# 87003697/DynamiCrafter

Hardware: AMD Instinct MI355X
Metric: frames/sec (and denoising-step ms), 16f@576x1024, DDIM 50 (higher is better)
Workload: dtype bf16; 1 GPU; inference_1024_v1.0.yaml: 1 clip/GPU, 16 frames, latent 72x128, DDIM 50 uniform_trailing eta=1, CFG 7.5 batched (cond+uncond), guidance_rescale 0.7, v-param+ZTSNR+dynamic rescale, hipGraph-captured step; clips_per_gpu=1, parallelism=dp1 over 1 distinct clips (no data-path collective), conditioning=local (1 rank), outputs_finite=True

## Files before the change

### dynamicrafter_amd/_hip.py

```python
import ctypes as C
import os
import threading

_HERE = os.path.dirname(os.path.abspath(__file__))
LIB_PATH = os.environ.get("DC_HIP_LIB") or os.path.join(_HERE, "csrc", "libdcrafter_hip.so")

DC_GEMM_OUT_F32 = 1
DC_GEMM_GEGLU = 2
DC_GEMM_GELU = 4


class DcGemmParams(C.Structure):
    _fields_ = [
        ("A", C.c_void_p), ("W", C.c_void_p), ("C", C.c_void_p), ("bias", C.c_void_p),
        ("rowvec", C.c_void_p), ("residual", C.c_void_p),
        ("lda", C.c_int), ("ldc", C.c_int), ("ldr", C.c_int), ("rowvec_ld", C.c_int),
        ("rows_per_vec", C.c_int),
        ("M", C.c_int), ("N", C.c_int), ("K", C.c_int), ("n_pad", C.c_int),
        ("mode", C.c_int), ("Cin", C.c_int),
        ("IH", C.c_int), ("IW", C.c_int), ("OH", C.c_int), ("OW", C.c_int),
        ("stride", C.c_int), ("pad", C.c_int), ("ups", C.c_int),
        ("T", C.c_int), ("HW", C.c_int),
        ("flags", C.c_int), ("alpha", C.c_float),
        ("workspace", C.c_void_p), ("workspace_bytes", C.c_longlong),
    ]


class DcDdimParams(C.Structure):
    _fields_ = [
        ("a_t", C.c_void_p), ("a_prev", C.c_void_p), ("sigma_t", C.c_void_p), ("sqrt_one_minus_at", C.c_void_p),
        ("sqrt_acp_t", C.c_void_p), ("sqrt_1macp_t", C.c_void_p), ("scale_ratio", C.c_void_p),
        ("step_index", C.c_void_p),
        ("index", C.c_int), ("v_param", C.c_int),
        ("cfg_scale", C.c_float), ("cfg_img", C.c_float), ("guidance_rescale", C.c_float),
        ("temperature", C.c_float),
        ("e_nchw", C.c_int), ("noise_step_stride", C.c_int64),
    ]


class DcDpmParams(C.Structure):
    _fields_ = [
        ("A", C.c_void_p), ("alpha_t", C.c_void_p), ("alpha_p_r", C.c_void_p), ("k", C.c_void_p), ("N", C.c_void_p),
        ("sqrt_one_minus_at", C.c_void_p), ("sqrt_acp_t", C.c_void_p), ("sqrt_1macp_t", C.c_void_p),
        ("scale_ratio", C.c_void_p), ("step_index", C.c_void_p),
        ("index", C.c_int), ("v_param", C.c_int),
        ("cfg_scale", C.c_float), ("cfg_img", C.c_float), ("guidance_rescale", C.c_float),
        ("temperature", C.c_float),
# ... 125 lines not shown
```

### dynamicrafter_amd/csrc/gemm_conv_glds.hip

```cpp
#include "dc_common.h"
#include "dcrafter_hip.h"
#include "lds_stage.h"
#include <stdint.h>
#include <stdlib.h>
#include <type_traits>
#include <utility>

namespace {

constexpr int GBM = 256;
constexpr int GBK = 64;
constexpr int GNT = 512;

struct GemmSplit {
    float* partial;
    int splits;
    int tile_begin;
    int tile_count;
    int* err;
    int whole;
};

template <int BN, bool GEGLU, int MODE, int GSTAGES>
__global__ __launch_bounds__(GNT) void gemm_conv_glds_kernel(const DcGemmParams p, const GemmSplit sp) {
    constexpr int NB = BN / 64;
    constexpr int BNOUT = GEGLU ? BN / 2 : BN;
    constexpr int A_BYTES = GBM * GBK * 2;
    constexpr int B_BYTES = BN * GBK * 2;
    constexpr int STAGE = A_BYTES + B_BYTES;
    constexpr int A_IT = 4;
    constexpr int B_IT = BN / 64;
    constexpr int LOADS = A_IT + B_IT;
    static_assert(GSTAGES == 2 || GSTAGES == 3, "ring depth");
    static_assert(!GEGLU || (NB % 2 == 0), "GEGLU needs value and gate blocks per wave");
    extern __shared__ __attribute__((aligned(16))) char smem[];

    const int tid = threadIdx.x;
    const int lane = tid & 63;
    const int wave = __builtin_amdgcn_readfirstlane(tid >> 6);
    const int wm = wave >> 1, wn = wave & 1;

    const int n_out = GEGLU ? (p.N >> 1) : p.N;
    const int tiles_n = (n_out + BNOUT - 1) / BNOUT;
    const int tiles_m = (p.M + GBM - 1) / GBM;
// ... 264 lines not shown
                    const uint2 rr = *reinterpret_cast<const uint2*>(p.residual + (size_t)m * p.ldr + n);
                    const float a0 = __uint_as_float(pk.x << 16) + __uint_as_float(rr.x << 16);
                    const float a1 = __uint_as_float(pk.x & 0xffff0000u) + __uint_as_float(rr.x & 0xffff0000u);
                    const float a2 = __uint_as_float(pk.y << 16) + __uint_as_float(rr.y << 16);
                    const float a3 = __uint_as_float(pk.y & 0xffff0000u) + __uint_as_float(rr.y & 0xffff0000u);
                    pk.x = pack_bf2(a0, a1);
                    pk.y = pack_bf2(a2, a3);
                }
                *reinterpret_cast<uint2*>(reinterpret_cast<bf16_t*>(p.C) + (size_t)m * p.ldc + n) = pk;
            }
        }
    }
}

template <int BN>
__global__ __launch_bounds__(256) void splitk_reduce_kernel(const DcGemmParams p, const GemmSplit sp) {
    constexpr int UPR = BN / 4;
    const int tiles_n = (p.N + BN - 1) / BN;
    const int t_loc = blockIdx.y;
    const int u = blockIdx.x * 256 + threadIdx.x;
    if (u >= GBM * UPR) return;
    const int r = u / UPR, c = (u - r * UPR) * 4;
    const int tile = sp.tile_begin + t_loc;
    const int m = (tile / tiles_n) * GBM + r, n = (tile % tiles_n) * BN + c;
    if (m >= p.M || n >= p.N) return;
    float4 v = make_float4(0.f, 0.f, 0.f, 0.f);
    for (int s = 0; s < sp.splits; ++s) {
        const float4 a = *reinterpret_cast<const float4*>(sp.partial + (((size_t)s * sp.tile_count + t_loc) * GBM + r) * BN + c);
        v.x += a.x; v.y += a.y; v.z += a.z; v.w += a.w;
    }
    if (p.bias) {
        const float4 bv = *reinterpret_cast<const float4*>(p.bias + n);
        v.x += bv.x; v.y += bv.y; v.z += bv.z; v.w += bv.w;
    }
    if (p.flags & DC_GEMM_GELU) { v.x = DC_GELU(v.x); v.y = DC_GELU(v.y); v.z = DC_GELU(v.z); v.w = DC_GELU(v.w); }
    if (p.rowvec) {
        const float4 rv = *reinterpret_cast<const float4*>(p.rowvec + (size_t)(m / p.rows_per_vec) * p.rowvec_ld + n);
        v.x += rv.x; v.y += rv.y; v.z += rv.z; v.w += rv.w;
    }
    if (p.alpha != 1.0f) { v.x *= p.alpha; v.y *= p.alpha; v.z *= p.alpha; v.w *= p.alpha; }
    if (p.flags & DC_GEMM_OUT_F32) {
        *reinterpret_cast<float4*>(reinterpret_cast<float*>(p.C) + (size_t)m * p.ldc + n) = v;
        return;
    }
    uint2 pk;
    pk.x = pack_bf2(v.x, v.y);
    pk.y = pack_bf2(v.z, v.w);
// ... 457 lines not shown
}

constexpr int PLAN_DEFAULT = 3 | 16;
constexpr int PLAN_MASK = 3 | 16 | 32 | 64 | 128 | 256;
inline bool plan_valid(int plan) { return plan >= 0 && plan <= 511 && !(plan & 4); }
std::atomic<int> g_gemm_plan{[] {
    const char* e = getenv("DC_GEMM_PLAN");
    const int v = e ? atoi(e) : PLAN_DEFAULT;
    return plan_valid(v) ? (v & PLAN_MASK) : PLAN_DEFAULT;
}()};
inline int pipe_min_k() { static const int v = [] { const char* e = getenv("DC_PIPE_MIN_K"); return e ? atoi(e) : 1920; }(); return v; }

template <int MODE, int EPI>
int launch_pipe_shape(const DcGemmParams& p, hipStream_t stream, GemmSplit sp, int gx, int gy) {
    sp.err = dc_error_word_device();
    if (!sp.err) return DC_ERR_ARG;
    return launch_pipe320x16<MODE, EPI>(p, stream, sp, gx, gy);
}

inline bool pipe_ok(const DcGemmParams& p, int plan) {
    if (!(plan & 3) || (!(plan & 2) && p.mode != 1)) return false;
    if (p.mode != 1 && p.K < pipe_min_k()) return false;
    if (p.flags & (DC_GEMM_GEGLU | DC_GEMM_OUT_F32)) return false;
    if (p.ups && !(p.mode == 1 && p.ups == 1 && p.stride == 1 && p.pad == 1 && p.OH == 2 * p.IH && p.OW == 2 * p.IW)) return false;
    if (p.N % 320 != 0 || p.n_pad < p.N || p.K % 64 != 0 || p.lda % 8 != 0 || ((uintptr_t)p.A % 16) != 0) return false;
    if (p.ldc % 8 != 0 || ((uintptr_t)p.C % 16) != 0 || (long long)p.M * p.ldc >= (1ll << 31)) return false;
    if (p.residual && (p.ldr % 8 != 0 || ((uintptr_t)p.residual % 16) != 0 || (long long)p.M * p.ldr >= (1ll << 31))) return false;
    long long rows = p.M, extra = 0;
    if (p.mode == 1) { if (p.Cin % 64 != 0 || p.K != 9 * p.Cin) return false; rows = (long long)(p.M / (p.OH * p.OW) + 1) * p.IH * p.IW; extra = 2ll * p.IW + 2; }
    else if (p.mode == 2) { if (p.Cin % 64 != 0 || p.K != 3 * p.Cin) return false; extra = 2ll * p.HW; }
    else if (p.mode != 0) return false;
    if ((rows + extra) * p.lda * 2 >= (1ll << 31)) return false;
    if (320ll * p.K * 2 >= (1ll << 31)) return false;
    return true;
}

int launch_pipe_whole(const DcGemmParams& p, hipStream_t stream) {
    const int ntiles = ((p.M + GBM - 1) / GBM) * (p.N / 320);
    GemmSplit sp;
    sp.partial = nullptr; sp.splits = 1; sp.tile_begin = 0; sp.tile_count = ntiles; sp.err = nullptr; sp.whole = 0;
    dc_note_variant(p.mode == 0 ? "gemm_pipe320x16_kernel" : p.mode == 2 ? "gemm_pipe320x16_kernel<tconv>"
                    : p.ups ? "gemm_pipe320x16_kernel<conv,ups>" : "gemm_pipe320x16_kernel<conv>");
    if (p.mode == 0) return p.residual ? launch_pipe_shape<0, 1>(p, stream, sp, ntiles, 1) : launch_pipe_shape<0, 0>(p, stream, sp, ntiles, 1);
    if (p.mode == 1 && p.ups) return p.residual ? launch_pipe_shape<3, 1>(p, stream, sp, ntiles, 1) : launch_pipe_shape<3, 0>(p, stream, sp, ntiles, 1);
    if (p.mode == 1) return p.residual ? launch_pipe_shape<1, 1>(p, stream, sp, ntiles, 1) : launch_pipe_shape<1, 0>(p, stream, sp, ntiles, 1);
    return p.residual ? launch_pipe_shape<2, 1>(p, stream, sp, ntiles, 1) : launch_pipe_shape<2, 0>(p, stream, sp, ntiles, 1);
}

template <int MODE, int BN = 320>
int launch_glds320_split(const DcGemmParams& p, hipStream_t stream, int ntiles, int full, int splits, bool use_pipe, bool merged) {
    constexpr int GSTAGES = 2;
    constexpr size_t lds = (size_t)GSTAGES * (GBM * GBK * 2 + BN * GBK * 2);
    static DcLdsOnce lds_once;
    if (const int e = lds_once.ensure(reinterpret_cast<const void*>(&gemm_conv_glds_kernel<BN, false, MODE, GSTAGES>), (int)lds)) return e;
    if constexpr (BN == 320) {
        if (use_pipe) {
            dc_note_variant(MODE == 0 ? "gemm_pipe320x16_kernel+splitk" : MODE == 2 ? "gemm_pipe320x16_kernel<tconv>+splitk"
                            : MODE == 3 ? "gemm_pipe320x16_kernel<conv,ups>+splitk" : "gemm_pipe320x16_kernel<conv>+splitk");
            GemmSplit sp;
            sp.err = nullptr; sp.whole = 0;
            if (full > 0 && merged && full % 8 == 0) {
                sp.partial = reinterpret_cast<float*>(p.workspace); sp.splits = splits; sp.tile_begin = full; sp.tile_count = ntiles - full;
                sp.whole = full;
                const int gx = full + sp.tile_count * splits;
                if (const int e = p.residual ? launch_pipe_shape<MODE, 1>(p, stream, sp, gx, 1) : launch_pipe_shape<MODE, 0>(p, stream, sp, gx, 1)) return e;
                sp.whole = 0;
            } else {
                if (full > 0) {
                    sp.partial = nullptr; sp.splits = 1; sp.tile_begin = 0; sp.tile_count = full;
                    if (const int e = p.residual ? launch_pipe_shape<MODE, 1>(p, stream, sp, full, 1) : launch_pipe_shape<MODE, 0>(p, stream, sp, full, 1)) return e;
                }
                sp.partial = reinterpret_cast<float*>(p.workspace); sp.splits = splits; sp.tile_begin = full; sp.tile_count = ntiles - full;
                if (const int e = launch_pipe_shape<MODE, 0>(p, stream, sp, sp.tile_count, splits)) return e;
            }
            hipLaunchKernelGGL((splitk_reduce_kernel<BN>), dim3((GBM * (BN / 4) + 255) / 256, sp.tile_count), dim3(256), 0, stream, p, sp);
            DC_CHECK_LAUNCH();
            return 0;
        }
    }
    if constexpr (BN == 320)
        dc_note_variant(MODE == 0 ? "gemm_conv_glds_kernel<320>+splitk" : MODE == 2 ? "gemm_conv_glds_kernel<320,tconv>+splitk" : "gemm_conv_glds_kernel<320,conv>+splitk");
    else
        dc_note_variant(MODE == 0 ? "gemm_conv_glds_kernel<256>+splitk" : MODE == 2 ? "gemm_conv_glds_kernel<256,tconv>+splitk" : "gemm_conv_glds_kernel<256,conv>+splitk");
    GemmSplit sp;
    sp.err = nullptr; sp.whole = 0;
    if (full > 0) {
        sp.partial = nullptr; sp.splits = 1; sp.tile_begin = 0; sp.tile_count = full;
        hipLaunchKernelGGL((gemm_conv_glds_kernel<BN, false, MODE, GSTAGES>), dim3(full), dim3(GNT), lds, stream, p, sp);
        DC_CHECK_LAUNCH();
    }
    sp.partial = reinterpret_cast<float*>(p.workspace); sp.splits = splits; sp.tile_begin = full; sp.tile_count = ntiles - full;
    hipLaunchKernelGGL((gemm_conv_glds_kernel<BN, false, MODE, GSTAGES>), dim3(sp.tile_count, splits), dim3(GNT), lds, stream, p, sp);
    DC_CHECK_LAUNCH();
    hipLaunchKernelGGL((splitk_reduce_kernel<BN>), dim3((GBM * (BN / 4) + 255) / 256, sp.tile_count), dim3(256), 0, stream, p, sp);
    DC_CHECK_LAUNCH();
    return 0;
}

template <int BN, int GSTAGES>
int launch_glds_mode(const DcGemmParams& p, hipStream_t stream) {
    if (p.mode == 0) return launch_glds<BN, false, 0, GSTAGES>(p, stream);
    if (p.mode == 1) return p.ups ? launch_glds<BN, false, 3, GSTAGES>(p, stream) : launch_glds<BN, false, 1, GSTAGES>(p, stream);
    return launch_glds<BN, false, 2, GSTAGES>(p, stream);
}

inline int persist_max_k() {
    static const int v = [] { const char* e = getenv("DC_GEMM_PERSIST_MAXK"); return e ? atoi(e) : 2560; }();
    return v;
}

inline float wave_eff(int wgs) { return (float)wgs / (float)(((wgs + 255) / 256) * 256); }

}

int dc_gemm_conv_glds_try(const DcGemmParams& p, hipStream_t stream) {
    const bool geglu = (p.flags & DC_GEMM_GEGLU) != 0;
    const int n_out = geglu ? p.N / 2 : p.N;
    const int tiles_m = (p.M + GBM - 1) / GBM;
    static const int force = [] { const char* e = getenv("DC_GEMM_TILE"); return e ? atoi(e) : 0; }();
    static const int persist = [] { const char* e = getenv("DC_GEMM_PERSIST"); return e ? atoi(e) : 1; }();
    if (geglu && p.mode != 0) return DC_ERR_ARG;
    const bool out_f32 = (p.flags & DC_GEMM_OUT_F32) != 0;
    const bool epi16 = out_f32 || ((n_out % 8 == 0) && (p.ldc % 8 == 0) && ((long long)p.M * p.ldc < (1ll << 31)) &&
                                   ((long long)p.M * p.ldr < (1ll << 31)) && ((uintptr_t)p.C % 16 == 0) &&
                                   (!p.residual || ((p.ldr % 8 == 0) && ((uintptr_t)p.residual % 16 == 0))));
    const int plan = g_gemm_plan.load(std::memory_order_relaxed);
    const bool use_pipe = pipe_ok(p, plan);
    const bool prefer_pipe = (force == 0) && use_pipe;
    if (persist && force == 0 && p.mode == 0 && epi16 && p.K <= persist_max_k() && !prefer_pipe) {
        static const int wide = [] { const char* e = getenv("DC_GEMM_PERSIST_WIDE"); return e ? atoi(e) : 1; }();
        if (geglu && (plan & 16) && ((plan & 32) || p.K <= 640) && pp_ok(p) && tiles_m * (n_out / 64) >= 1024) return launch_pp(p, stream);
        if (geglu) {
            if (wide && n_out % 128 == 0 && tiles_m * (n_out / 128) >= 512) return launch_persist<256, true>(p, stream, 256);
            const int nt = tiles_m * (n_out / 64);
            if (nt >= 512) return launch_persist<128, true>(p, stream, 256);
        } else {
            if (wide && p.N % 320 == 0 && p.n_pad >= p.N && tiles_m * (p.N / 320) >= 512)
                return launch_persist<320, false>(p, stream, 256);
            const int t128n = (p.N + 127) / 128;
            const float waste = (float)(t128n * 128) / (float)p.N;
            if (waste <= 1.15f && tiles_m * t128n >= 512) return launch_persist<128, false>(p, stream, 256);
            const int t64n = (p.N + 63) / 64;
            if (waste > 1.15f && tiles_m * t64n >= 512) return launch_persist<64, false>(p, stream, 256);
        }
    }
    static const int persist_conv_maxk = [] { const char* e = getenv("DC_GEMM_PERSIST_CONV_MAXK"); return e ? atoi(e) : 2880; }();
    if (persist && force == 0 && !prefer_pipe && !geglu && !out_f32 && epi16 && (p.mode == 2 || (p.mode == 1 && !p.ups)) &&
        p.N % 320 == 0 && p.n_pad >= p.N && tiles_m * (p.N / 320) >= (p.mode == 1 ? 1024 : 512) && p.K <= persist_conv_maxk)
        return launch_persist_conv320(p, stream);
    if (geglu) {
        const int w256 = (n_out % 128 == 0 && p.n_pad >= p.N) ? tiles_m * (n_out / 128) : 0;
        const int w128 = tiles_m * (n_out / 64);
        if ((force == 256 || (force == 0 && w256 >= 512 && wave_eff(w256) > 0.8f)) && w256 > 0)
            return launch_glds<256, true, 0, 2>(p, stream);
        if (w128 < 384) return -100;
        return launch_glds<128, true, 0, 3>(p, stream);
    }
    const int t128 = (p.N + 127) / 128;
    const bool n320 = (p.N % 320 == 0) && (p.n_pad >= p.N);
    const int w320 = n320 ? tiles_m * (p.N / 320) : 0;
    const int w128 = tiles_m * t128;
    const float waste128 = (float)(t128 * 128) / (float)p.N;
    const bool pipe_conv = use_pipe && p.mode == 1 && force == 0;
    float s320 = n320 ? (pipe_conv ? 1.4f : 1.25f) * wave_eff(w320) : 0.f;
    float s128 = wave_eff(w128) / waste128;
    if (w320 < (pipe_conv ? 128 : 200)) s320 = 0.f;
    if (w128 < 384) s128 = 0.f;
    static const int splitk = [] { const char* e = getenv("DC_GEMM_SPLITK"); return e ? atoi(e) : 1; }();
    if (splitk && force == 0 && n320 && p.workspace && p.n_pad >= p.N) {
        const int nk = p.K / GBK;
        int full = 0, splits = 0;
        if (w320 < 200 && w320 >= 8) {
            splits = 256 / w320;
            if (splits > 12) splits = 12;
            while (splits > 2 && nk / splits < 12) --splits;
        } else if (w320 > 256 && w320 <= 1280 && (w320 % 256) != 0 && (w320 % 256) <= 128) {
            full = (w320 / 256) * 256;
            splits = 256 / (w320 - full);
            if (splits > 8) splits = 8;
            while (splits > 2 && nk / splits < 8) --splits;
        }
        const size_t need = (size_t)splits * (size_t)(w320 - full) * GBM * 320 * sizeof(float);
        if (splits >= 2 && nk / splits >= (full ? 8 : 12) && need <= (size_t)p.workspace_bytes) {
            const bool merged = !(plan & 64);
            if (p.mode == 0) return launch_glds320_split<0>(p, stream, w320, full, splits, use_pipe, merged);
            if (p.mode == 1) return p.ups ? launch_glds320_split<3>(p, stream, w320, full, splits, use_pipe, merged)
                                          : launch_glds320_split<1>(p, stream, w320, full, splits, use_pipe, merged);
            return launch_glds320_split<2>(p, stream, w320, full, splits, use_pipe, merged);
        }
    }
    static const int splitk256 = [] { const char* e = getenv("DC_GEMM_SPLITK256"); return e ? atoi(e) : 1; }();
    if (splitk && splitk256 && force == 0 && !n320 && !out_f32 && p.workspace && p.N % 256 == 0 && p.n_pad >= p.N && (p.mode != 1 || !p.ups)) {
        const int w256s = tiles_m * (p.N / 256), nk = p.K / GBK;
        if (w256s > 256 && w256s <= 1280 && (w256s % 256) != 0 && (w256s % 256) <= 128) {
            const int full = (w256s / 256) * 256;
            int splits = 256 / (w256s - full);
            if (splits > 8) splits = 8;
            while (splits > 2 && nk / splits < 8) --splits;
            const size_t need = (size_t)splits * (size_t)(w256s - full) * GBM * 256 * sizeof(float);
            if (splits >= 2 && nk / splits >= 8 && need <= (size_t)p.workspace_bytes) {
                if (p.mode == 0) return launch_glds320_split<0, 256>(p, stream, w256s, full, splits, false, false);
                if (p.mode == 1) return launch_glds320_split<1, 256>(p, stream, w256s, full, splits, false, false);
                return launch_glds320_split<2, 256>(p, stream, w256s, full, splits, false, false);
            }
        }
    }
// ... 17 lines not shown
```

### dynamicrafter_amd/csrc/gemm_pipe16.h

```cpp
#pragma once

typedef __attribute__((ext_vector_type(4))) float gp_f32x4_t;

#define GP16_MFMA_A(d, w, x) asm volatile("v_mfma_f32_16x16x32_bf16 %0, %1, %2, %0" : "+a"(d) : "v"(w), "v"(x))
#define GP16_MFMA_V(d, w, x) asm volatile("v_mfma_f32_16x16x32_bf16 %0, %1, %2, %0" : "+v"(d) : "v"(w), "v"(x))

__device__ __forceinline__ void gp16_settle(gp_f32x4_t (&acc)[4][20]) {
#pragma unroll
    for (int rb = 0; rb < 4; ++rb)
        asm volatile("s_nop 7\n\ts_nop 7"
                     : "+a"(acc[rb][0]), "+a"(acc[rb][1]), "+a"(acc[rb][2]), "+a"(acc[rb][3]), "+a"(acc[rb][4]), "+a"(acc[rb][5]),
                       "+a"(acc[rb][6]), "+a"(acc[rb][7]), "+a"(acc[rb][8]), "+a"(acc[rb][9]), "+a"(acc[rb][10]), "+a"(acc[rb][11]),
                       "+a"(acc[rb][12]), "+a"(acc[rb][13]), "+a"(acc[rb][14]), "+a"(acc[rb][15]), "+v"(acc[rb][16]), "+v"(acc[rb][17]),
                       "+v"(acc[rb][18]), "+v"(acc[rb][19]));
    asm volatile("s_nop 7\n\ts_nop 7" ::: "memory");
}

template <int MODE, int EPI>
__global__ __launch_bounds__(256, 1) __attribute__((amdgpu_waves_per_eu(1, 1)))
void gemm_pipe320x16_kernel(const DcGemmParams p, const GemmSplit sp) {
    extern __shared__ __attribute__((aligned(16))) char smem[];
    const int tid = threadIdx.x, lane = tid & 63;
    const int wave = __builtin_amdgcn_readfirstlane(tid >> 6);
    const int lr = lane & 15, lq = lane >> 4;

    const int tiles_n = p.N / 320;
    int bx = blockIdx.x, by = blockIdx.y, tile_begin = sp.tile_begin, tile_count = sp.tile_count, nsplit = sp.splits;
    float* partial = sp.partial;
    if (sp.whole > 0) {
        if (bx < sp.whole) { tile_begin = 0; tile_count = sp.whole; nsplit = 1; partial = nullptr; by = 0; }
        else { bx -= sp.whole; by = bx / tile_count; bx -= by * tile_count; }
    }
    const int swz = tile_begin + xcd_remap(bx, tile_count);
    const int tile_n = swz % tiles_n;
    const int tile_m = swz / tiles_n;
    const int m0 = tile_m * GBM;
    const int n0 = tile_n * 320;

    const int nk_all = p.K / GBK;
    const int kt_lo = (int)(((long long)by * nk_all) / nsplit);
    const int kt_hi = (int)(((long long)(by + 1) * nk_all) / nsplit);
    const int nk = kt_hi - kt_lo;

    lds_int_t* const cnt_landed = (lds_int_t*)(smem + GP_CNT);
    lds_int_t* const cnt_freed = cnt_landed + 1;
    if (tid < 2) cnt_landed[tid] = 0;
    __syncthreads();
    int gave_up = 0;

    const unsigned lda2 = (unsigned)p.lda * 2u;
    unsigned rowoff[4];
    int mask[4];
    long long bias = 0;
    if (MODE == 1) bias = (long long)(p.pad * p.IW + p.pad) * lda2;
    if (MODE == 2) bias = (long long)p.HW * lda2;
    if (MODE == 3) bias = (long long)(p.IW + 1) * lda2;
#ifdef GP_DBG_QUAD_ROWS
    const int lr_a = lr & ~3, lq_a = lane & 3;
#else
    const int lr_a = lr, lq_a = lq;
#endif
#pragma unroll
    for (int rb = 0; rb < 4; ++rb) {
        const int m = m0 + wave * 64 + rb * 16 + lr_a;
        const bool ok = m < p.M;
        const int mm = ok ? m : 0;
        if (MODE == 0) {
            rowoff[rb] = (unsigned)mm * lda2 + lq_a * 16;
            mask[rb] = ok ? 1 : 0;
        } else if (MODE == 1) {
            const int ohw = p.OH * p.OW;
            const int n = mm / ohw;
            const int rem = mm - n * ohw;
            const int oy = rem / p.OW;
            const int ox = rem - oy * p.OW;
            const int iy0 = oy * p.stride - p.pad, ix0 = ox * p.stride - p.pad;
            int mk = 0;
#pragma unroll
            for (int t = 0; t < 9; ++t) {
                const int iy = iy0 + t / 3, ix = ix0 + t % 3;
                if (ok && iy >= 0 && iy < p.IH && ix >= 0 && ix < p.IW) mk |= 1 << t;
            }
            mask[rb] = mk;
            rowoff[rb] = (unsigned)(((n * p.IH + iy0 + p.pad) * p.IW + ix0 + p.pad)) * lda2 + lq_a * 16;
        } else if (MODE == 3) {
            const int ohw = p.OH * p.OW;
            const int n = mm / ohw;
            const int rem = mm - n * ohw;
            const int oy = rem / p.OW;
            const int ox = rem - oy * p.OW;
            int mk = 0;
#pragma unroll
            for (int t = 0; t < 9; ++t) {
                const int uy = oy + t / 3 - 1, ux = ox + t % 3 - 1;
                if (ok && uy >= 0 && uy < p.OH && ux >= 0 && ux < p.OW) mk |= 1 << t;
            }
            mask[rb] = mk | ((oy & 1) << 9) | ((ox & 1) << 10);
            rowoff[rb] = (unsigned)(((n * p.IH + (oy >> 1) + 1) * p.IW + (ox >> 1) + 1)) * lda2 + lq_a * 16;
        } else {
            const int frame = (mm / p.HW) % p.T;
            int mk = 0;
#pragma unroll
            for (int t = 0; t < 3; ++t) {
                const int tt = frame + t - 1;
                if (ok && tt >= 0 && tt < p.T) mk |= 1 << t;
            }
            mask[rb] = mk;
            rowoff[rb] = (unsigned)mm * lda2 + lq_a * 16;
        }
    }
    gp_i32x4_t ars;
    {
        const unsigned long long ab = (unsigned long long)(uintptr_t)p.A - (unsigned long long)bias;
        ars[0] = __builtin_amdgcn_readfirstlane((int)(unsigned)ab);
        ars[1] = __builtin_amdgcn_readfirstlane((int)(unsigned)((ab >> 32) & 0xffffu));
        ars[2] = 0x7fffffff;
        ars[3] = 0x00020000;
    }
    auto a_tile = [&](int kt, unsigned (&vo)[4], int& soff) __attribute__((always_inline)) {
        int tap = 0;
        if (MODE == 0) {
            soff = kt * 128;
        } else if (MODE == 1) {
            const int cs = kt / 9;
            tap = kt - cs * 9;
            const int dy = tap / 3, dx = tap - dy * 3;
            soff = (dy * p.IW + dx) * (int)lda2 + cs * 128;
        } else if (MODE == 3) {
            const int cs = kt / 9;
            tap = kt - cs * 9;
            const int dy = tap / 3, dx = tap - dy * 3;
            soff = cs * 128;
            const int y0 = dy == 0 ? -p.IW * (int)lda2 : 0, y1 = dy == 2 ? p.IW * (int)lda2 : 0;
            const int x0 = dx == 0 ? -(int)lda2 : 0, x1 = dx == 2 ? (int)lda2 : 0;
#pragma unroll
            for (int rb = 0; rb < 4; ++rb) {
                const unsigned o = rowoff[rb] + (unsigned)(((mask[rb] >> 9) & 1) ? y1 : y0) + (unsigned)(((mask[rb] >> 10) & 1) ? x1 : x0);
                vo[rb] = ((mask[rb] >> tap) & 1) ? o : 0x80000000u;
            }
            return;
        } else {
            const int cs = kt / 3;
            tap = kt - cs * 3;
            soff = tap * p.HW * (int)lda2 + cs * 128;
        }
#pragma unroll
        for (int rb = 0; rb < 4; ++rb) vo[rb] = ((mask[rb] >> tap) & 1) ? rowoff[rb] : 0x80000000u;
    };

    const unsigned lds_base = (unsigned)(uintptr_t)((const lds_char_t*)smem);
    unsigned voffB[10];
#pragma unroll
    for (int j = 0; j < 10; ++j) {
        const int row = (j * 4 + wave) * 8 + (lane >> 3);
        voffB[j] = (unsigned)row * (unsigned)p.K * 2u + (unsigned)(((lane & 7) ^ (((wave & 1) * 4 + (lane >> 4)) & 7)) << 4);
        asm volatile("" : "+v"(voffB[j]));
    }
    auto w_src = [&](int kt) __attribute__((always_inline)) -> unsigned long long {
        return (unsigned long long)(uintptr_t)p.W + ((unsigned long long)n0 * p.K + (unsigned long long)kt * 64) * 2ull;
    };

    unsigned bofs[3][2];
#pragma unroll
    for (int st = 0; st < 3; ++st)
#pragma unroll
        for (int s = 0; s < 2; ++s) {
            bofs[st][s] = lds_base + st * GP_STAGE + lr * 128 + (((4 * s + lq) ^ ((lr >> 1) & 7)) << 4);
            asm volatile("" : "+v"(bofs[st][s]));
        }
    bf16x8_t Bf[5];
    auto rd_b = [&](int slot, unsigned addr, int cb) __attribute__((always_inline)) {
        Bf[slot] = *(lds_vfrag_t*)((const lds_char_t*)(uintptr_t)addr + cb * 2048);
    };

    u32x4_t A[3][4][2];
    gp_f32x4_t acc[4][20];
#pragma unroll
    for (int i = 0; i < 4; ++i)
#pragma unroll
        for (int j = 0; j < 20; ++j)
#pragma unroll
            for (int r = 0; r < 4; ++r) acc[i][j][r] = 0.f;
// ... 113 lines not shown

    if (partial) {
        const size_t slot = (size_t)by * tile_count + (size_t)(swz - tile_begin);
        float* const dst = partial + (slot * GBM + wave * 64 + lr) * 320 + 4 * lq;
#pragma unroll
        for (int rb = 0; rb < 4; ++rb)
#pragma unroll
            for (int cb = 0; cb < 20; ++cb)
                *reinterpret_cast<float4*>(dst + (size_t)rb * 16 * 320 + cb * 16) = make_float4(acc[rb][cb][0], acc[rb][cb][1], acc[rb][cb][2], acc[rb][cb][3]);
        return;
    }
    char* const ebuf = smem + GP_RING + wave * 2048;
    int lane_e = lane;
    asm volatile("" : "+v"(lane_e));
    const int er = lane_e & 15, eq = lane_e >> 4;
    const int rrow = lane_e >> 2, rc = lane_e & 3;
    const char* const rbase = reinterpret_cast<const char*>(p.residual);
    char* const cbase = reinterpret_cast<char*>(p.C);
#pragma unroll
    for (int rb = 0; rb < 4; ++rb) {
        const int m_acc = m0 + wave * 64 + rb * 16 + er;
        const float* rv = p.rowvec ? p.rowvec + (size_t)((m_acc < p.M ? m_acc : 0) / p.rows_per_vec) * p.rowvec_ld : nullptr;
        int mr = m0 + wave * 64 + rb * 16 + rrow;
        const bool rok = mr < p.M;
        if (!rok) mr = p.M - 1;
        const unsigned co = ((unsigned)mr * (unsigned)p.ldc + (unsigned)(n0 + rc * 8)) * 2u;
        const unsigned ro = ((unsigned)mr * (unsigned)p.ldr + (unsigned)(n0 + rc * 8)) * 2u;
#pragma unroll
        for (int cp = 0; cp < 10; ++cp) {
            u32x4_t rr;
            if constexpr (EPI == 1) rr = *reinterpret_cast<const u32x4_t*>(rbase + ro + cp * 64);
#pragma unroll
            for (int h = 0; h < 2; ++h) {
                const int cb = 2 * cp + h;
                const int n = n0 + cb * 16 + 4 * eq;
                float4 v = make_float4(acc[rb][cb][0], acc[rb][cb][1], acc[rb][cb][2], acc[rb][cb][3]);
                if (p.bias) {
                    const float4 bv = *reinterpret_cast<const float4*>(p.bias + n);
                    v.x += bv.x; v.y += bv.y; v.z += bv.z; v.w += bv.w;
                }
                if (p.flags & DC_GEMM_GELU) { v.x = DC_GELU(v.x); v.y = DC_GELU(v.y); v.z = DC_GELU(v.z); v.w = DC_GELU(v.w); }
                if (rv) {
                    const float4 r4 = *reinterpret_cast<const float4*>(rv + n);
                    v.x += r4.x; v.y += r4.y; v.z += r4.z; v.w += r4.w;
                }
                if (p.alpha != 1.0f) { v.x *= p.alpha; v.y *= p.alpha; v.z *= p.alpha; v.w *= p.alpha; }
                uint2 pk;
                pk.x = pack_bf2(v.x, v.y);
// ... 25 lines not shown
```

### dynamicrafter_amd/lvdm/modules/networks/openaimodel3d.py

```python
import math

import torch
import torch.nn as nn

from .... import ops
from ....ops import PackedWeight
from ....param_tree import attach_params

import os

_BF16 = torch.bfloat16
_FF_FUSED = os.environ.get("DC_FF_FUSED", "1") != "0"
_LN_FUSED = os.environ.get("DC_LN_FUSED", "1") != "0"
_LR_FUSED = os.environ.get("DC_LR_FUSED", "1") != "0"
_TA_FUSED = os.environ.get("DC_TA_FUSED", "1") != "0"
_TA_FUSED_C = tuple(int(k) for k in os.environ.get("DC_TA_FUSED_C", "320,640").split(","))
_FFP_FUSED = os.environ.get("DC_FFP_FUSED", "1") != "0"
_TC_FUSED = os.environ.get("DC_TC_FUSED", "1") != "0"
_FUSED_MIN_ROWS = int(os.environ.get("DC_FUSED_MIN_ROWS", "4096"))
_LN_FUSED_K = tuple(int(k) for k in os.environ.get("DC_LN_FUSED_K", "320,640").split(","))
C_IN_PAD = 64


def _block_layout(cfg):
# ... 284 lines not shown
                elif kind == "res":
                    d = {"gn1": (f32(p + ".in_layers.0.weight"), f32(p + ".in_layers.0.bias")),
                         "conv1": PackedWeight.conv3x3(self._p(p + ".in_layers.2.weight"), self._p(p + ".in_layers.2.bias"), device),
                         "emb": lin(p + ".emb_layers.1"),
                         "gn2": (f32(p + ".out_layers.0.weight"), f32(p + ".out_layers.0.bias")),
                         "conv2": PackedWeight.conv3x3(self._p(p + ".out_layers.3.weight"), self._p(p + ".out_layers.3.bias"), device)}
                    if a["cin"] != a["cout"]:
                        d["skip"] = lin(p + ".skip_connection")
                    if a["tconv"]:
                        d["tc"] = []
                        for i, ci in ((1, 2), (2, 3), (3, 3), (4, 3)):
                            q = f"{p}.temopral_conv.conv{i}"
                            d["tc"].append(((f32(q + ".0.weight"), f32(q + ".0.bias")),
                                            PackedWeight.tconv3(self._p(f"{q}.{ci}.weight"), self._p(f"{q}.{ci}.bias"), device)))
                    out.append(d)
                elif kind == "spatial":
                    out.append(with_projp({"norm": (f32(p + ".norm.weight"), f32(p + ".norm.bias")), "proj_in": lin(p + ".proj_in"),
                                           "blk": tblock(p + ".transformer_blocks.0", True), "proj_out": lin(p + ".proj_out")}, p))
                elif kind == "temporal":
                    out.append(temporal(p))
                elif kind == "down":
                    out.append({"conv": PackedWeight.conv3x3(self._p(p + ".op.weight"), self._p(p + ".op.bias"), device)})
                elif kind == "up":
                    out.append({"conv": PackedWeight.conv3x3(self._p(p + ".conv.weight"), self._p(p + ".conv.bias"), device)})
            return out

        down_path, middle, up_path = self._layout
        P["in"] = [pack_block(f"input_blocks.{i}", b) for i, b in enumerate(down_path)]
        P["mid"] = pack_block("middle_block", middle)
        P["out"] = [pack_block(f"output_blocks.{i}", b) for i, b in enumerate(up_path)]
        P["out_gn"] = (f32("out.0.weight"), f32("out.0.bias"))
        P["out_conv"] = PackedWeight.conv3x3(self._p("out.2.weight"), self._p("out.2.bias"), device, n_align=4)
        P["device"] = device
        self._pack_gen = getattr(self, "_pack_gen", 0) + 1
        P["gen"] = self._pack_gen
        return P

    def packed(self, device):
        if self._packed is None or self._packed["device"] != device:
            self._packed = self._pack(device)
        return self._packed

    def _gn(self, x, wb, tag, *, n_inst, rpi, eps, silu):
        y = self._arena.get(tag, x.shape[0], x.shape[1], device=x.device)
        return ops.groupnorm(x, y, wb[0], wb[1], groups=32, n_inst=n_inst, rows_per_inst=rpi, eps=eps, silu=silu)

    def _ln(self, x, wb, tag):
# ... 331 lines not shown
```

### dynamicrafter_amd/ops.py

```python
import ctypes as C
import os
import math

import torch

from . import _hip
from ._hip import DcDdimParams, DcGemmParams, check

_BF16 = torch.bfloat16


def stream_ptr():
    return C.c_void_p(torch.cuda.current_stream().cuda_stream)


class Tracer:

    def __init__(self):
        self.records = []

    def __enter__(self):
        global _TRACE
        _TRACE = self
        return self
# ... 36 lines not shown
    e0, e1 = tr._event(), tr._event()
    sp = stream_ptr()
    l.dc_event_record(e0, sp)
    check(fn(*args), name)
    l.dc_event_record(e1, sp)
    if name == "dc_gemm_conv":
        name = l.dc_gemm_last_variant().decode()
    tr.records.append((name, flops, nbytes, e0, e1, tag))


def _ptr(t):
    return C.c_void_p(0 if t is None else t.data_ptr())


def _rows(t, name="tensor", dtype=_BF16):
    if t.dtype != dtype or t.dim() != 2 or t.stride(1) != 1 or not t.is_cuda:
        raise ValueError(f"{name}: expected CUDA {dtype} rows [R, C] with unit column stride, got "
                         f"{t.dtype} {tuple(t.shape)} strides {t.stride()} on {t.device}")
    return t


class PackedWeight:

    __slots__ = ("w", "bias", "N", "K", "n_pad", "Cin", "taps", "k_real")

    def __init__(self, w, bias, N, K, Cin, taps, k_real=None):
        self.w, self.bias, self.N, self.K, self.Cin, self.taps = w, bias, N, K, Cin, taps
        self.n_pad = w.shape[0]
        self.k_real = k_real

    @staticmethod
    def _finish(w2d, bias, device, Cin, taps, pad_n_to=None):
        N, K = w2d.shape
        n_pad = (N + 127) // 128 * 128
        if pad_n_to is not None:
            n_pad = max(n_pad, pad_n_to)
        wp = torch.zeros((n_pad, K), dtype=_BF16, device=device)
        wp[:N] = w2d.to(device=device, dtype=_BF16)
        b = None if bias is None else bias.detach().to(device=device, dtype=torch.float32).contiguous()
        return PackedWeight(wp, b, N, K, Cin, taps)

    @staticmethod
    def linear(weight, bias, device, n_align=1):
        w = weight.detach().reshape(weight.shape[0], -1)
        N, K = w.shape
        if K % 64 != 0:
            kp = (K + 63) // 64 * 64
            w = torch.nn.functional.pad(w, (0, kp - K))
        if N % n_align != 0:
            npad = (N + n_align - 1) // n_align * n_align
            w = torch.nn.functional.pad(w, (0, 0, 0, npad - N))
            if bias is not None:
                bias = torch.nn.functional.pad(bias.detach(), (0, npad - N))
        return PackedWeight._finish(w, bias, device, w.shape[1], 1)

    @staticmethod
    def conv3x3(weight, bias, device, n_align=1):
        co, ci = weight.shape[0], weight.shape[1]
        w = weight.detach().permute(0, 2, 3, 1)
        cip = (ci + 63) // 64 * 64
        if cip != ci:
            w = torch.nn.functional.pad(w, (0, cip - ci))
        w = w.reshape(co, 9, cip // 64, 64).permute(0, 2, 1, 3).reshape(co, 9 * cip)
        if co % n_align != 0:
            npad = (co + n_align - 1) // n_align * n_align
            w = torch.nn.functional.pad(w, (0, 0, 0, npad - co))
            if bias is not None:
                bias = torch.nn.functional.pad(bias.detach(), (0, npad - co))
        pw = PackedWeight._finish(w, bias, device, cip, 9)
        pw.k_real = 9 * ci
        return pw

    @staticmethod
    def conv3x3_c8_as_linear(weight, bias, device):
        co, ci = weight.shape[0], weight.shape[1]
        assert ci <= 8
        w = torch.zeros(co, 16, 8, dtype=weight.dtype)
        w[:, :9, :ci] = weight.detach().permute(0, 2, 3, 1).reshape(co, 9, ci)
        pw = PackedWeight._finish(w.reshape(co, 128), bias, device, 128, 1)
        pw.k_real = 9 * ci
        return pw

    @staticmethod
    def tconv3(weight, bias, device):
        co, ci = weight.shape[0], weight.shape[1]
        assert ci % 64 == 0, "temporal conv width must be a multiple of 64"
        w = weight.detach().reshape(co, ci // 64, 64, 3).permute(0, 1, 3, 2).reshape(co, 3 * ci)
        return PackedWeight._finish(w, bias, device, ci, 3)


def gemm(a, pw, out, *, M=None, residual=None, rowvec=None, rows_per_vec=1, geglu=False, gelu=False, alpha=1.0,
         conv=None, tconv=None):
    _rows(a, "a")
# ... 3 lines not shown
    p = DcGemmParams()
    p.A, p.W, p.C = a.data_ptr(), pw.w.data_ptr(), out.data_ptr()
    p.bias = 0 if pw.bias is None else pw.bias.data_ptr()
    p.rowvec = 0 if rowvec is None else rowvec.data_ptr()
    p.rowvec_ld = 0 if rowvec is None else rowvec.stride(0)
    p.rows_per_vec = rows_per_vec
    p.residual = 0 if residual is None else _rows(residual, "residual").data_ptr()
    p.ldr = 0 if residual is None else residual.stride(0)
    p.lda, p.ldc = a.stride(0), out.stride(0)
    p.M = out.shape[0] if M is None else M
    p.N, p.K, p.n_pad = pw.N, pw.K, pw.n_pad
    p.Cin = pw.Cin
    p.flags = (_hip.DC_GEMM_OUT_F32 if out_f32 else 0) | (_hip.DC_GEMM_GEGLU if geglu else 0) | \
        (_hip.DC_GEMM_GELU if gelu else 0)
    p.alpha = alpha
    ws = _gemm_workspace(a.device, torch.cuda.current_stream().cuda_stream)
    p.workspace, p.workspace_bytes = ws.data_ptr(), ws.numel()
    if conv is not None:
        p.mode = 1
        p.IH, p.IW, p.OH, p.OW = conv["IH"], conv["IW"], conv["OH"], conv["OW"]
        p.stride, p.pad, p.ups = conv.get("stride", 1), conv.get("pad", 1), conv.get("ups", 0)
        if pw.taps != 9 or a.shape[1] < pw.Cin:
            raise ValueError("conv3x3 weight / activation mismatch")
    elif tconv is not None:
        p.mode = 2
        p.T, p.HW = tconv["T"], tconv["HW"]
        if pw.taps != 3:
            raise ValueError("tconv weight mismatch")
    else:
        p.mode = 0
        if a.shape[1] < pw.K:
            raise ValueError(f"gemm: activation has {a.shape[1]} columns, weight K={pw.K}")
    n_out = pw.N // 2 if geglu else pw.N
    if out.shape[1] < n_out:
        raise ValueError(f"gemm: out has {out.shape[1]} columns, need {n_out}")
    if out.shape[0] < p.M or (residual is not None and (residual.shape[0] < p.M or residual.shape[1] < n_out)):
        raise ValueError(f"gemm: out/residual have fewer than M={p.M} rows (or residual fewer than {n_out} columns)")
    if p.mode == 1:
        if p.M % (p.OH * p.OW) != 0 or a.shape[0] < (p.M // (p.OH * p.OW)) * p.IH * p.IW:
            raise ValueError(f"conv3x3: M={p.M} output rows need {p.M // (p.OH * p.OW)} frames of {p.IH}x{p.IW} input rows, "
                             f"activation has {a.shape[0]}")
    elif a.shape[0] < p.M:
        raise ValueError(f"gemm: activation has {a.shape[0]} rows, M={p.M}")
    if p.mode == 2 and (p.M % (p.T * p.HW) != 0 or a.shape[1] < pw.Cin):
        raise ValueError("tconv: M must be a multiple of T*HW and the activation at least Cin wide")
    if rowvec is not None and (rowvec.shape[0] * rows_per_vec < p.M or rowvec.shape[1] < n_out):
# ... 826 lines not shown
```

### include/dcrafter_hip.h

```cpp
#ifndef DCRAFTER_HIP_H
#define DCRAFTER_HIP_H
#include <stdint.h>

#ifdef __cplusplus
extern "C" {
#endif

#define DC_ERR_SHAPE (-1)
#define DC_ERR_ARG   (-2)

#define DC_GEMM_OUT_F32 1
#define DC_GEMM_GEGLU   2
#define DC_GEMM_GELU    4

typedef struct DcGemmParams {
    const uint16_t* A;
    const uint16_t* W;
    void* C;
    const float* bias;
    const float* rowvec;
    const uint16_t* residual;
    int lda, ldc, ldr, rowvec_ld;
    int rows_per_vec;
    int M, N, K, n_pad;
    int mode;
    int Cin;
    int IH, IW, OH, OW;
    int stride, pad, ups;
    int T, HW;
    int flags;
    float alpha;
    void* workspace;
    long long workspace_bytes;
} DcGemmParams;

const char* dc_gemm_last_variant(void);

int dc_gemm_set_plan(int plan);

int64_t dc_gemm_workspace_bytes(void);

int dc_gemm_conv(const DcGemmParams* p, void* stream);

int dc_groupnorm(const uint16_t* x, int ldx, uint16_t* y, int ldy, const float* gamma, const float* beta,
                 int C, int groups, int n_inst, int rows_per_inst, float eps, int silu,
                 float* workspace, void* stream);
int64_t dc_groupnorm_workspace_bytes(int n_inst, int groups, int rows_per_inst);

int dc_layernorm(const uint16_t* x, int ldx, uint16_t* y, int ldy, const float* gamma, const float* beta,
                 int rows, int C, float eps, void* stream);

int dc_flash_attn_d64(const uint16_t* q, const uint16_t* k, const uint16_t* v, uint16_t* o,
                      int ldq, int ldk, int ldv, int ldo, int batch, int heads, int Lq, int Lk,
                      int64_t q_bstride, int64_t kv_bstride, float scale, int accumulate, float acc_scale,
                      void* stream);

// ... 210 lines not shown
```

Baseline: 2.602 frames/s.

## Fold nearest-upsample into conv3x3 via per-phase 2x2 weights

Replaces the upsample-then-3x3-conv path with a sub-pixel phase decomposition. Each of the four output phases uses a 2x2 effective kernel applied directly to the low-resolution input. The summed weights are split into bf16 hi/lo pairs, giving 7 taps per input channel instead of 9, and the kernel scatters each phase's rows back to the interleaved output. This cuts the K dimension of the upsample convolutions. The cost is a second precomputed weight tensor, new phase indexing in the pipe kernel, and a numeric change from summing the weights before rounding.

Result: no change. 2.609 frames/s, median of 6 (+0.2%).

```diff
diff --git a/dynamicrafter_amd/_hip.py b/dynamicrafter_amd/_hip.py
--- a/dynamicrafter_amd/_hip.py
+++ b/dynamicrafter_amd/_hip.py
@@ -23,6 +23,7 @@
         ("T", C.c_int), ("HW", C.c_int),
         ("flags", C.c_int), ("alpha", C.c_float),
         ("workspace", C.c_void_p), ("workspace_bytes", C.c_longlong),
+        ("W_phase", C.c_void_p),
     ]
 
 
diff --git a/dynamicrafter_amd/csrc/gemm_conv_glds.hip b/dynamicrafter_amd/csrc/gemm_conv_glds.hip
--- a/dynamicrafter_amd/csrc/gemm_conv_glds.hip
+++ b/dynamicrafter_amd/csrc/gemm_conv_glds.hip
@@ -19,7 +19,10 @@
     int tile_count;
     int* err;
     int whole;
+    int phases = 0;
 };
+
+constexpr int UPS_PHASES = 2;
 
 template <int BN, bool GEGLU, int MODE, int GSTAGES>
 __global__ __launch_bounds__(GNT) void gemm_conv_glds_kernel(const DcGemmParams p, const GemmSplit sp) {
@@ -330,7 +333,15 @@
     if (u >= GBM * UPR) return;
     const int r = u / UPR, c = (u - r * UPR) * 4;
     const int tile = sp.tile_begin + t_loc;
-    const int m = (tile / tiles_n) * GBM + r, n = (tile % tiles_n) * BN + c;
+    int m = (tile / tiles_n) * GBM + r;
+    const int n = (tile % tiles_n) * BN + c;
+    if (sp.phases) {
+        const int tm = tile / tiles_n, ph = tm & 3, ihw = p.IH * p.IW;
+        const int ml = (tm >> 2) * GBM + r;
+        if (ml >= (p.M >> 2)) return;
+        const int f = ml / ihw, rem = ml - f * ihw, y = rem / p.IW, x = rem - y * p.IW;
+        m = (f * p.OH + 2 * y + (ph >> 1)) * p.OW + 2 * x + (ph & 1);
+    }
     if (m >= p.M || n >= p.N) return;
     float4 v = make_float4(0.f, 0.f, 0.f, 0.f);
     for (int s = 0; s < sp.splits; ++s) {
@@ -834,12 +845,17 @@
     if (!(plan & 3) || (!(plan & 2) && p.mode != 1)) return false;
     if (p.mode != 1 && p.K < pipe_min_k()) return false;
     if (p.flags & (DC_GEMM_GEGLU | DC_GEMM_OUT_F32)) return false;
-    if (p.ups && !(p.mode == 1 && p.ups == 1 && p.stride == 1 && p.pad == 1 && p.OH == 2 * p.IH && p.OW == 2 * p.IW)) return false;
+    const bool phases = p.ups == UPS_PHASES;
+    if (p.ups && !(p.mode == 1 && (p.ups == 1 || phases) && p.stride == 1 && p.pad == 1 && p.OH == 2 * p.IH && p.OW == 2 * p.IW)) return false;
     if (p.N % 320 != 0 || p.n_pad < p.N || p.K % 64 != 0 || p.lda % 8 != 0 || ((uintptr_t)p.A % 16) != 0) return false;
     if (p.ldc % 8 != 0 || ((uintptr_t)p.C % 16) != 0 || (long long)p.M * p.ldc >= (1ll << 31)) return false;
     if (p.residual && (p.ldr % 8 != 0 || ((uintptr_t)p.residual % 16) != 0 || (long long)p.M * p.ldr >= (1ll << 31))) return false;
     long long rows = p.M, extra = 0;
-    if (p.mode == 1) { if (p.Cin % 64 != 0 || p.K != 9 * p.Cin) return false; rows = (long long)(p.M / (p.OH * p.OW) + 1) * p.IH * p.IW; extra = 2ll * p.IW + 2; }
+    if (p.mode == 1) {
+        if (p.Cin % 64 != 0 || p.K != (phases ? 7 : 9) * p.Cin) return false;
+        rows = (long long)(p.M / (p.OH * p.OW) + 1) * p.IH * p.IW;
+        extra = phases ? p.IW + 1ll : 2ll * p.IW + 2;
+    }
     else if (p.mode == 2) { if (p.Cin % 64 != 0 || p.K != 3 * p.Cin) return false; extra = 2ll * p.HW; }
     else if (p.mode != 0) return false;
     if ((rows + extra) * p.lda * 2 >= (1ll << 31)) return false;
@@ -851,6 +867,11 @@
     const int ntiles = ((p.M + GBM - 1) / GBM) * (p.N / 320);
     GemmSplit sp;
     sp.partial = nullptr; sp.splits = 1; sp.tile_begin = 0; sp.tile_count = ntiles; sp.err = nullptr; sp.whole = 0;
+    if (p.mode == 1 && p.ups == UPS_PHASES) {
+        dc_note_variant("gemm_pipe320x16_kernel<conv,ups>/phases");
+        sp.phases = 1;
+        return launch_pipe_shape<4, 0>(p, stream, sp, ntiles, 1);
+    }
     dc_note_variant(p.mode == 0 ? "gemm_pipe320x16_kernel" : p.mode == 2 ? "gemm_pipe320x16_kernel<tconv>"
                     : p.ups ? "gemm_pipe320x16_kernel<conv,ups>" : "gemm_pipe320x16_kernel<conv>");
     if (p.mode == 0) return p.residual ? launch_pipe_shape<0, 1>(p, stream, sp, ntiles, 1) : launch_pipe_shape<0, 0>(p, stream, sp, ntiles, 1);
@@ -859,18 +880,19 @@
     return p.residual ? launch_pipe_shape<2, 1>(p, stream, sp, ntiles, 1) : launch_pipe_shape<2, 0>(p, stream, sp, ntiles, 1);
 }
 
+template <int MODE, int BN>
+int launch_glds320_split_8wave(const DcGemmParams& p, hipStream_t stream, int ntiles, int full, int splits);
+
 template <int MODE, int BN = 320>
 int launch_glds320_split(const DcGemmParams& p, hipStream_t stream, int ntiles, int full, int splits, bool use_pipe, bool merged) {
-    constexpr int GSTAGES = 2;
-    constexpr size_t lds = (size_t)GSTAGES * (GBM * GBK * 2 + BN * GBK * 2);
-    static DcLdsOnce lds_once;
-    if (const int e = lds_once.ensure(reinterpret_cast<const void*>(&gemm_conv_glds_kernel<BN, false, MODE, GSTAGES>), (int)lds)) return e;
+    static_assert(MODE != 4 || BN == 320, "the phase form exists on the one-wave kernel only");
     if constexpr (BN == 320) {
         if (use_pipe) {
             dc_note_variant(MODE == 0 ? "gemm_pipe320x16_kernel+splitk" : MODE == 2 ? "gemm_pipe320x16_kernel<tconv>+splitk"
-                            : MODE == 3 ? "gemm_pipe320x16_kernel<conv,ups>+splitk" : "gemm_pipe320x16_kernel<conv>+splitk");
+                            : MODE == 3 ? "gemm_pipe320x16_kernel<conv,ups>+splitk"
+                            : MODE == 4 ? "gemm_pipe320x16_kernel<conv,ups>/phases+splitk" : "gemm_pipe320x16_kernel<conv>+splitk");
             GemmSplit sp;
-            sp.err = nullptr; sp.whole = 0;
+            sp.err = nullptr; sp.whole = 0; sp.phases = MODE == 4 ? 1 : 0;
             if (full > 0 && merged && full % 8 == 0) {
                 sp.partial = reinterpret_cast<float*>(p.workspace); sp.splits = splits; sp.tile_begin = full; sp.tile_count = ntiles - full;
                 sp.whole = full;
@@ -890,6 +912,16 @@
             return 0;
         }
     }
+    if constexpr (MODE == 4) return DC_ERR_ARG;
+    else return launch_glds320_split_8wave<MODE, BN>(p, stream, ntiles, full, splits);
+}
+
+template <int MODE, int BN>
+int launch_glds320_split_8wave(const DcGemmParams& p, hipStream_t stream, int ntiles, int full, int splits) {
+    constexpr int GSTAGES = 2;
+    constexpr size_t lds = (size_t)GSTAGES * (GBM * GBK * 2 + BN * GBK * 2);
+    static DcLdsOnce lds_once;
+    if (const int e = lds_once.ensure(reinterpret_cast<const void*>(&gemm_conv_glds_kernel<BN, false, MODE, GSTAGES>), (int)lds)) return e;
     if constexpr (BN == 320)
         dc_note_variant(MODE == 0 ? "gemm_conv_glds_kernel<320>+splitk" : MODE == 2 ? "gemm_conv_glds_kernel<320,tconv>+splitk" : "gemm_conv_glds_kernel<320,conv>+splitk");
     else
@@ -919,6 +951,32 @@
 inline int persist_max_k() {
     static const int v = [] { const char* e = getenv("DC_GEMM_PERSIST_MAXK"); return e ? atoi(e) : 2560; }();
     return v;
+}
+
+inline bool split_plan320(int w320, int nk, long long workspace_bytes, int& full, int& splits) {
+    full = 0; splits = 0;
+    if (w320 < 200 && w320 >= 8) {
+        splits = 256 / w320;
+        if (splits > 12) splits = 12;
+        while (splits > 2 && nk / splits < 12) --splits;
+    } else if (w320 > 256 && w320 <= 1280 && (w320 % 256) != 0 && (w320 % 256) <= 128) {
+        full = (w320 / 256) * 256;
+        splits = 256 / (w320 - full);
+        if (splits > 8) splits = 8;
+        while (splits > 2 && nk / splits < 8) --splits;
+    }
+    const size_t need = (size_t)splits * (size_t)(w320 - full) * GBM * 320 * sizeof(float);
+    return splits >= 2 && nk / splits >= (full ? 8 : 12) && need <= (size_t)workspace_bytes;
+}
+
+inline bool ups_phase_ok(const DcGemmParams& p, int plan, DcGemmParams& q) {
+    static const int on = [] { const char* e = getenv("DC_UPS_PHASES"); return e ? atoi(e) : 1; }();
+    if (!on || !p.W_phase || !(plan & 1) || p.mode != 1 || p.ups != 1) return false;
+    if (p.residual || p.rowvec || (p.flags & DC_GEMM_OUT_F32)) return false;
+    if (p.M % (4 * GBM) != 0 || ((uintptr_t)p.W_phase % 16) != 0) return false;
+    q = p;
+    q.W = p.W_phase; q.W_phase = nullptr; q.K = 7 * p.Cin; q.ups = UPS_PHASES;
+    return pipe_ok(q, plan);
 }
 
 inline float wave_eff(int wgs) { return (float)wgs / (float)(((wgs + 255) / 256) * 256); }
@@ -939,6 +997,15 @@
     const int plan = g_gemm_plan.load(std::memory_order_relaxed);
     const bool use_pipe = pipe_ok(p, plan);
     const bool prefer_pipe = (force == 0) && use_pipe;
+    static const int splitk = [] { const char* e = getenv("DC_GEMM_SPLITK"); return e ? atoi(e) : 1; }();
+    DcGemmParams q;
+    if (force == 0 && ups_phase_ok(p, plan, q)) {
+        const int w320 = tiles_m * (p.N / 320);
+        int full = 0, splits = 0;
+        if (splitk && p.workspace && split_plan320(w320, q.K / GBK, p.workspace_bytes, full, splits))
+            return launch_glds320_split<4>(q, stream, w320, full, splits, true, !(plan & 64));
+        return launch_pipe_whole(q, stream);
+    }
     if (persist && force == 0 && p.mode == 0 && epi16 && p.K <= persist_max_k() && !prefer_pipe) {
         static const int wide = [] { const char* e = getenv("DC_GEMM_PERSIST_WIDE"); return e ? atoi(e) : 1; }();
         if (geglu && (plan & 16) && ((plan & 32) || p.K <= 640) && pp_ok(p) && tiles_m * (n_out / 64) >= 1024) return launch_pp(p, stream);
@@ -978,22 +1045,9 @@
     float s128 = wave_eff(w128) / waste128;
     if (w320 < (pipe_conv ? 128 : 200)) s320 = 0.f;
     if (w128 < 384) s128 = 0.f;
-    static const int splitk = [] { const char* e = getenv("DC_GEMM_SPLITK"); return e ? atoi(e) : 1; }();
     if (splitk && force == 0 && n320 && p.workspace && p.n_pad >= p.N) {
-        const int nk = p.K / GBK;
         int full = 0, splits = 0;
-        if (w320 < 200 && w320 >= 8) {
-            splits = 256 / w320;
-            if (splits > 12) splits = 12;
-            while (splits > 2 && nk / splits < 12) --splits;
-        } else if (w320 > 256 && w320 <= 1280 && (w320 % 256) != 0 && (w320 % 256) <= 128) {
-            full = (w320 / 256) * 256;
-            splits = 256 / (w320 - full);
-            if (splits > 8) splits = 8;
-            while (splits > 2 && nk / splits < 8) --splits;
-        }
-        const size_t need = (size_t)splits * (size_t)(w320 - full) * GBM * 320 * sizeof(float);
-        if (splits >= 2 && nk / splits >= (full ? 8 : 12) && need <= (size_t)p.workspace_bytes) {
+        if (split_plan320(w320, p.K / GBK, p.workspace_bytes, full, splits)) {
             const bool merged = !(plan & 64);
             if (p.mode == 0) return launch_glds320_split<0>(p, stream, w320, full, splits, use_pipe, merged);
             if (p.mode == 1) return p.ups ? launch_glds320_split<3>(p, stream, w320, full, splits, use_pipe, merged)
diff --git a/dynamicrafter_amd/csrc/gemm_pipe16.h b/dynamicrafter_amd/csrc/gemm_pipe16.h
--- a/dynamicrafter_amd/csrc/gemm_pipe16.h
+++ b/dynamicrafter_amd/csrc/gemm_pipe16.h
@@ -34,7 +34,8 @@
     const int swz = tile_begin + xcd_remap(bx, tile_count);
     const int tile_n = swz % tiles_n;
     const int tile_m = swz / tiles_n;
-    const int m0 = tile_m * GBM;
+    const int phase = MODE == 4 ? __builtin_amdgcn_readfirstlane(tile_m & 3) : 0;
+    const int m0 = (MODE == 4 ? (tile_m >> 2) : tile_m) * GBM;
     const int n0 = tile_n * 320;
 
     const int nk_all = p.K / GBK;
@@ -54,7 +55,7 @@
     long long bias = 0;
     if (MODE == 1) bias = (long long)(p.pad * p.IW + p.pad) * lda2;
     if (MODE == 2) bias = (long long)p.HW * lda2;
-    if (MODE == 3) bias = (long long)(p.IW + 1) * lda2;
+    if (MODE == 3 || MODE == 4) bias = (long long)(p.IW + 1) * lda2;
 #ifdef GP_DBG_QUAD_ROWS
     const int lr_a = lr & ~3, lq_a = lane & 3;
 #else
@@ -63,7 +64,7 @@
 #pragma unroll
     for (int rb = 0; rb < 4; ++rb) {
         const int m = m0 + wave * 64 + rb * 16 + lr_a;
-        const bool ok = m < p.M;
+        const bool ok = MODE == 4 ? m < (p.M >> 2) : m < p.M;
         const int mm = ok ? m : 0;
         if (MODE == 0) {
             rowoff[rb] = (unsigned)mm * lda2 + lq_a * 16;
@@ -97,6 +98,21 @@
             }
             mask[rb] = mk | ((oy & 1) << 9) | ((ox & 1) << 10);
             rowoff[rb] = (unsigned)(((n * p.IH + (oy >> 1) + 1) * p.IW + (ox >> 1) + 1)) * lda2 + lq_a * 16;
+        } else if (MODE == 4) {
+            const int ihw = p.IH * p.IW;
+            const int n = mm / ihw;
+            const int rem = mm - n * ihw;
+            const int y = rem / p.IW;
+            const int x = rem - y * p.IW;
+            const int sy0 = y + (phase >> 1) - 1, sx0 = x + (phase & 1) - 1;
+            int mk = 0;
+#pragma unroll
+            for (int t = 0; t < 4; ++t) {
+                const int sy = sy0 + (t >> 1), sx = sx0 + (t & 1);
+                if (ok && sy >= 0 && sy < p.IH && sx >= 0 && sx < p.IW) mk |= 1 << t;
+            }
+            mask[rb] = mk;
+            rowoff[rb] = (unsigned)(((n * p.IH + sy0 + 1) * p.IW + sx0 + 1)) * lda2 + lq_a * 16;
         } else {
             const int frame = (mm / p.HW) % p.T;
             int mk = 0;
@@ -139,6 +155,12 @@
                 vo[rb] = ((mask[rb] >> tap) & 1) ? o : 0x80000000u;
             }
             return;
+        } else if (MODE == 4) {
+            const int cs = kt / 7;
+            const int j = kt - cs * 7;
+            const int o = (j - 1) >> 1;
+            tap = j == 0 ? phase : o + (o >= phase ? 1 : 0);
+            soff = ((tap >> 1) * p.IW + (tap & 1)) * (int)lda2 + cs * 128;
         } else {
             const int cs = kt / 3;
             tap = kt - cs * 3;
@@ -157,7 +179,8 @@
         asm volatile("" : "+v"(voffB[j]));
     }
     auto w_src = [&](int kt) __attribute__((always_inline)) -> unsigned long long {
-        return (unsigned long long)(uintptr_t)p.W + ((unsigned long long)n0 * p.K + (unsigned long long)kt * 64) * 2ull;
+        const unsigned long long wrow = MODE == 4 ? (unsigned long long)phase * (unsigned long long)p.n_pad + (unsigned long long)n0 : (unsigned long long)n0;
+        return (unsigned long long)(uintptr_t)p.W + (wrow * p.K + (unsigned long long)kt * 64) * 2ull;
     };
 
     unsigned bofs[3][2];
@@ -317,8 +340,16 @@
         const int m_acc = m0 + wave * 64 + rb * 16 + er;
         const float* rv = p.rowvec ? p.rowvec + (size_t)((m_acc < p.M ? m_acc : 0) / p.rows_per_vec) * p.rowvec_ld : nullptr;
         int mr = m0 + wave * 64 + rb * 16 + rrow;
-        const bool rok = mr < p.M;
-        if (!rok) mr = p.M - 1;
+        const bool rok = MODE == 4 ? mr < (p.M >> 2) : mr < p.M;
+        if (MODE == 4) {
+            if (!rok) mr = 0;
+            const int ihw = p.IH * p.IW;
+            const int n = mr / ihw;
+            const int rem = mr - n * ihw;
+            const int y = rem / p.IW;
+            const int x = rem - y * p.IW;
+            mr = (n * p.OH + 2 * y + (phase >> 1)) * p.OW + 2 * x + (phase & 1);
+        } else if (!rok) mr = p.M - 1;
         const unsigned co = ((unsigned)mr * (unsigned)p.ldc + (unsigned)(n0 + rc * 8)) * 2u;
         const unsigned ro = ((unsigned)mr * (unsigned)p.ldr + (unsigned)(n0 + rc * 8)) * 2u;
 #pragma unroll
diff --git a/dynamicrafter_amd/lvdm/modules/networks/openaimodel3d.py b/dynamicrafter_amd/lvdm/modules/networks/openaimodel3d.py
--- a/dynamicrafter_amd/lvdm/modules/networks/openaimodel3d.py
+++ b/dynamicrafter_amd/lvdm/modules/networks/openaimodel3d.py
@@ -330,7 +330,7 @@
                 elif kind == "down":
                     out.append({"conv": PackedWeight.conv3x3(self._p(p + ".op.weight"), self._p(p + ".op.bias"), device)})
                 elif kind == "up":
-                    out.append({"conv": PackedWeight.conv3x3(self._p(p + ".conv.weight"), self._p(p + ".conv.bias"), device)})
+                    out.append({"conv": PackedWeight.conv3x3_ups(self._p(p + ".conv.weight"), self._p(p + ".conv.bias"), device)})
             return out
 
         down_path, middle, up_path = self._layout
diff --git a/dynamicrafter_amd/ops.py b/dynamicrafter_amd/ops.py
--- a/dynamicrafter_amd/ops.py
+++ b/dynamicrafter_amd/ops.py
@@ -82,12 +82,13 @@
 
 class PackedWeight:
 
-    __slots__ = ("w", "bias", "N", "K", "n_pad", "Cin", "taps", "k_real")
+    __slots__ = ("w", "bias", "N", "K", "n_pad", "Cin", "taps", "k_real", "w_phase")
 
     def __init__(self, w, bias, N, K, Cin, taps, k_real=None):
         self.w, self.bias, self.N, self.K, self.Cin, self.taps = w, bias, N, K, Cin, taps
         self.n_pad = w.shape[0]
         self.k_real = k_real
+        self.w_phase = None
 
     @staticmethod
     def _finish(w2d, bias, device, Cin, taps, pad_n_to=None):
@@ -129,6 +130,30 @@
                 bias = torch.nn.functional.pad(bias.detach(), (0, npad - co))
         pw = PackedWeight._finish(w, bias, device, cip, 9)
         pw.k_real = 9 * ci
+        return pw
+
+    @staticmethod
+    def conv3x3_ups(weight, bias, device):
+        pw = PackedWeight.conv3x3(weight, bias, device)
+        co, ci = weight.shape[0], weight.shape[1]
+        w = weight.detach().to(_BF16).to(torch.float64)
+        S = torch.tensor([[[1, 0, 0], [0, 1, 1]], [[1, 1, 0], [0, 0, 1]]], dtype=torch.float64, device=w.device)
+        ph = torch.einsum("pad,qbe,ocde->pqabco", S, S, w)
+        ph = ph.permute(0, 1, 5, 2, 3, 4).reshape(4, co, 4, ci)
+        hi = ph.to(_BF16)
+        lo = (ph - hi.to(torch.float64)).to(_BF16)
+        cip = pw.Cin
+        parts = torch.zeros(4, co, 7, cip, dtype=_BF16, device=w.device)
+        for p in range(4):
+            assert not bool(lo[p, :, p].any())
+            parts[p, :, 0, :ci] = hi[p, :, p]
+            for o, t in enumerate(t for t in range(4) if t != p):
+                parts[p, :, 1 + 2 * o, :ci] = hi[p, :, t]
+                parts[p, :, 2 + 2 * o, :ci] = lo[p, :, t]
+        parts = parts.reshape(4, co, 7, cip // 64, 64).permute(0, 1, 3, 2, 4).reshape(4, co, 7 * cip)
+        wp = torch.zeros((4, pw.n_pad, 7 * cip), dtype=_BF16, device=device)
+        wp[:, :co] = parts.to(device=device)
+        pw.w_phase = wp
         return pw
 
     @staticmethod
@@ -178,6 +203,8 @@
         p.stride, p.pad, p.ups = conv.get("stride", 1), conv.get("pad", 1), conv.get("ups", 0)
         if pw.taps != 9 or a.shape[1] < pw.Cin:
             raise ValueError("conv3x3 weight / activation mismatch")
+        if pw.w_phase is not None and p.ups == 1:
+            p.W_phase = pw.w_phase.data_ptr()
     elif tconv is not None:
         p.mode = 2
         p.T, p.HW = tconv["T"], tconv["HW"]
diff --git a/include/dcrafter_hip.h b/include/dcrafter_hip.h
--- a/include/dcrafter_hip.h
+++ b/include/dcrafter_hip.h
@@ -32,6 +32,7 @@
     float alpha;
     void* workspace;
     long long workspace_bytes;
+    const uint16_t* W_phase;
 } DcGemmParams;
 
 const char* dc_gemm_last_variant(void);
```
